# yangdongchao/RSTnet

Hardware: NVIDIA H100
Metric: codec_frames_per_s (higher is better)
Workload: dtype f32

## Files before the change

rstnet_b200/csrc/gemm_tc.cu:

```cuda
#include <cstdlib>

#include "common.cuh"
#include "tc_common.cuh"
#include "../../include/rstnet_b200.h"

namespace rstnet {
extern void count_launch();
using namespace tc;

constexpr int TC_BM = 128;
constexpr int TC_BKE = 32;
constexpr int TC_A_BYTES = TC_BM * 128;
constexpr int TC_CONSUMER_WARPS = 8;
constexpr int TC_THREADS = 32 * TC_CONSUMER_WARPS + 32;
constexpr int TC_CHUNK_STAGES = 4;

struct TcParams {
  float* C;
  float* C2;
  int act2;
  long long c_i_stride, c_o_stride, c_split_stride;
  const float* R;
  long long r_i_stride, r_o_stride, r_split_stride;
  const float* bias;
  const float* scale;
  int n_split;
  int I_out, O_out, N, Kc;
  int taps, tap_di, tap_do, o_mul, kchunks;
  int pre_act, post_act, i_tiles;
  int m_tiles, n_tiles;
};

template <int BN, int PREC>
struct TcCfg {
  static constexpr bool SPLIT = PREC == 0;
  static constexpr int B_BYTES = BN * 128;
  static constexpr int STAGE_BYTES = TC_A_BYTES + B_BYTES * (SPLIT ? 2 : 1);
  static constexpr int STAGES = (200 * 1024 / STAGE_BYTES) > 8 ? 8 : (200 * 1024 / STAGE_BYTES);
  static constexpr int SMEM_BYTES = STAGES * STAGE_BYTES + 1024  + 256 ;
};

__device__ __forceinline__ float tf32_rna(float x) {
  const uint32_t u = __float_as_uint(x);
  return __uint_as_float((x != x ? u | 0x00400000u : u + 0x1000u) & 0xFFFFE000u);
}
__device__ __forceinline__ float tf32_rna_lo(float x, float hi) {
  const float d = x - hi;
  return d != d ? 0.f : __uint_as_float((__float_as_uint(d) + 0x1000u) & 0xFFFFE000u);
}

__device__ __forceinline__ float act_tc(float x, int act) {
  if (act == ACT_ELU) return elu_fast(x);
  if (act == ACT_GELU) return gelu_f(x);
  return x;
}

template <bool SPLIT, bool PRE_ELU>
__device__ __forceinline__ void tc_build_a(uint32_t st, uint32_t a_row, uint32_t a_sw, uint32_t (&ah)[4][4], uint32_t (&al)[4][4]) {
#pragma unroll
  for (int k = 0; k < 4; ++k) {
#pragma unroll
    for (int e = 0; e < 4; ++e) {
      const uint32_t chunk = (uint32_t)(2 * k + (e >> 1));
      float v;
      asm volatile("ld.shared.f32 %0, [%1];" : "=f"(v) : "r"(st + a_row + (e & 1) * 1024u + ((chunk ^ a_sw) << 4)));
      if (PRE_ELU) {
        const float e = __expf(v) - 1.f;
        v = v > 0.f ? v : e;
      }
      if (SPLIT) {
        const bool nonfinite = !(fabsf(v) < INFINITY);
        const float h = nonfinite ? 0.f : __uint_as_float((__float_as_uint(v) + 0x1000u) & 0xFFFFE000u);
        const float d = v - h;
        ah[k][e] = __float_as_uint(h);
        al[k][e] = (__float_as_uint(d) + (nonfinite ? 0u : 0x1000u)) & 0xFFFFE000u;
      } else {
        ah[k][e] = __float_as_uint(tf32_rna(v));
      }
    }
  }
}

template <int BN, bool SPLIT>
__device__ __forceinline__ void tc_mma_stage(float (&d0)[BN / 2], float (&d1)[BN / 2], const uint32_t (&ah)[4][4],
                                             const uint32_t (&al)[4][4], uint64_t db, uint64_t dbl, bool first) {
#pragma unroll
  for (int k = 0; k < 4; ++k) {
    const uint32_t acc_in = (first && k == 0) ? 0u : 1u;
    wgmma_tf32_rs<BN>(d0, ah[k], db + (uint64_t)(2 * k), acc_in);
    if (SPLIT) {
      wgmma_tf32_rs<BN>(d1, al[k], db + (uint64_t)(2 * k), acc_in);
      wgmma_tf32_rs<BN>(d1, ah[k], dbl + (uint64_t)(2 * k), 1u);
    }
  }
}

template <int BN, int PREC, bool PRE_ELU>
__global__ void __launch_bounds__(TC_THREADS, 1)
gemm_tc_kernel(const __grid_constant__ CUtensorMap tmA, const __grid_constant__ CUtensorMap tmW,
               const __grid_constant__ CUtensorMap tmWlo, const TcParams p) {
  using Cfg = TcCfg<BN, PREC>;
  constexpr int S = Cfg::STAGES;
  constexpr int CH = TC_CHUNK_STAGES;
  constexpr int NR = BN / 2;
  extern __shared__ uint8_t smem_raw[];
  uint8_t* smem = smem_raw + ((1024u - (smem_u32(smem_raw) & 1023u)) & 1023u);
  uint64_t* full = reinterpret_cast<uint64_t*>(smem + S * Cfg::STAGE_BYTES);
  uint64_t* empty = full + S;
  const int warp = threadIdx.x / 32, lane = threadIdx.x % 32;
  const int total_k = p.taps * p.kchunks;
  const int total_tiles = p.m_tiles * p.n_tiles;

  if (threadIdx.x == 0) {
    for (int s = 0; s < S; ++s) {
      mbar_init(&full[s], 1);
      mbar_init(&empty[s], TC_CONSUMER_WARPS);
    }
    fence_barrier_init();
  }
  __syncthreads();

  if (warp == TC_CONSUMER_WARPS) {
    if (elect_one()) {
      tma_prefetch_desc(&tmA);
      tma_prefetch_desc(&tmW);
      if (Cfg::SPLIT) tma_prefetch_desc(&tmWlo);
      int g = 0;
      for (int t = blockIdx.x; t < total_tiles; t += gridDim.x) {
        const int nt = t % p.n_tiles, mt = t / p.n_tiles;
        const int i0 = (mt % p.i_tiles) * TC_BM, ot = mt / p.i_tiles, n0 = nt * BN;
        for (int kit = 0; kit < total_k; ++kit, ++g) {
          const int s = g % S;
          mbar_wait(&empty[s], ((g / S) & 1) ^ 1);
          const int tap = kit / p.kchunks, kc = kit % p.kchunks;
          uint8_t* st = smem + s * Cfg::STAGE_BYTES;
          mbar_arrive_expect_tx(&full[s], Cfg::STAGE_BYTES);
          tma_load_3d(st, &tmA, &full[s], kc * TC_BKE, i0 + tap * p.tap_di, ot * p.o_mul + tap * p.tap_do);
          tma_load_2d(st + TC_A_BYTES, &tmW, &full[s], kit * TC_BKE, n0);
          if (Cfg::SPLIT) tma_load_2d(st + TC_A_BYTES + Cfg::B_BYTES, &tmWlo, &full[s], kit * TC_BKE, n0);
        }
      }
    }
    return;
  }

  const int wg = warp / 4, wq = warp % 4, gq = lane / 4, tq = lane % 4;
  const int r0 = wg * 64 + wq * 16 + gq;
  const uint32_t a_row = (uint32_t)r0 * 128u + (uint32_t)tq * 4u, a_sw = (uint32_t)(r0 & 7);
  const uint32_t smem0 = smem_u32(smem);
  float acc[NR], d0[NR], d1[NR];
#pragma unroll
  for (int j = 0; j < NR; ++j) d0[j] = d1[j] = 0.f;
  int g = 0;
  for (int t = blockIdx.x; t < total_tiles; t += gridDim.x) {
    const int nt = t % p.n_tiles, mt = t / p.n_tiles;
    const int i0 = (mt % p.i_tiles) * TC_BM, ot = mt / p.i_tiles, n0 = nt * BN;
#pragma unroll
    for (int j = 0; j < NR; ++j) acc[j] = 0.f;
    for (int k0 = 0; k0 < total_k; k0 += CH) {
      const int nst = total_k - k0 < CH ? total_k - k0 : CH;
      for (int u = 0; u < nst; ++u, ++g) {
        const int s = g % S;
        mbar_wait(&full[s], (g / S) & 1);
        const uint32_t st = smem0 + (uint32_t)(s * Cfg::STAGE_BYTES);
        uint32_t ah[4][4], al[4][4];
        tc_build_a<Cfg::SPLIT, PRE_ELU>(st, a_row, a_sw, ah, al);
        const uint64_t db = gmma_desc_sw128(st + TC_A_BYTES);
        const uint64_t dbl = gmma_desc_sw128(st + TC_A_BYTES + Cfg::B_BYTES);
        wgmma_fence();
        tc_mma_stage<BN, Cfg::SPLIT>(d0, d1, ah, al, db, dbl, u == 0);
        wgmma_commit();
        wgmma_wait<0>();
        __syncwarp();
        if (lane == 0) mbar_arrive(&empty[s]);
      }
      fence_acc(d0);
      if (Cfg::SPLIT) fence_acc(d1);
#pragma unroll
      for (int j = 0; j < NR; ++j) acc[j] += Cfg::SPLIT ? d0[j] + d1[j] : d0[j];
    }
#pragma unroll
    for (int h = 0; h < 2; ++h) {
      const int i = i0 + r0 + 8 * h;
      if (i >= p.I_out) continue;
      float* crow = p.C + (long long)ot * p.c_o_stride + (long long)i * p.c_i_stride;
      float* crow2 = p.C2 ? p.C2 + (long long)ot * p.c_o_stride + (long long)i * p.c_i_stride : nullptr;
      const float* rrow = p.R ? p.R + (long long)ot * p.r_o_stride + (long long)i * p.r_i_stride : nullptr;
#pragma unroll
      for (int b = 0; b < BN / 8; ++b) {
        const int n = n0 + 8 * b + 2 * tq;
        if (n < p.N) {
          float2 v = make_float2(acc[4 * b + 2 * h], acc[4 * b + 2 * h + 1]);
          if (p.bias) {
            const float2 bb = *reinterpret_cast<const float2*>(p.bias + n);
            v.x += bb.x; v.y += bb.y;
          }
          if (p.scale) {
            const float2 ss = *reinterpret_cast<const float2*>(p.scale + n);
            v.x *= ss.x; v.y *= ss.y;
          }
          long long coff = n, roff = n;
          if (p.n_split > 0) {
            const int j = n / p.n_split, co = n % p.n_split;
            coff = (long long)j * p.c_split_stride + co;
            roff = (long long)j * p.r_split_stride + co;
          }
          if (rrow) {
            const float2 rr = *reinterpret_cast<const float2*>(rrow + roff);
            v.x += rr.x; v.y += rr.y;
          }
          if (crow2)
            *reinterpret_cast<float2*>(crow2 + coff) = make_float2(act_tc(v.x, p.act2), act_tc(v.y, p.act2));
          *reinterpret_cast<float2*>(crow + coff) = make_float2(act_tc(v.x, p.post_act), act_tc(v.y, p.post_act));
        }
      }
    }
  }
}

constexpr int RB_B_BYTES = 64 * 128;
constexpr int RB_STAGE_BYTES = TC_A_BYTES + 2 * RB_B_BYTES;
constexpr int RB_STAGES = 6;

struct RbParams {
  float* out;
  long long o_i_stride, o_o_stride;
  const float* b1;
  const float* b2;
  int I_out, i_tiles, m_tiles;
};

template <int C>
struct RbCfg {
  static constexpr int N1 = C / 2;
  static constexpr int KCH = C / 32;
  static constexpr int P1 = 3 * KCH;
  static constexpr int NS = C / 64;
  static constexpr int K2 = N1 / 32;
  static constexpr int H_BYTES = K2 * TC_A_BYTES;
  static constexpr int SMEM_BYTES = RB_STAGES * RB_STAGE_BYTES + H_BYTES + 1024  + 256 ;
  static constexpr bool ring_ok() {
    for (int j = 0; j < NS; ++j)
      for (int kc = 0; kc < KCH; ++kc)
        if ((P1 + j) % RB_STAGES == (2 * KCH + kc) % RB_STAGES) return false;
    return RB_STAGES >= KCH + NS;
  }
  static_assert(ring_ok(), "ring too small for the held residual stages");
  static_assert(K2 * 2 * RB_B_BYTES <= RB_STAGE_BYTES, "a phase-2 slice must fit one stage");
};

template <int C>
__global__ void __launch_bounds__(TC_THREADS, 1)
resblock_tc_kernel(const __grid_constant__ CUtensorMap tmY, const __grid_constant__ CUtensorMap tmW1,
                   const __grid_constant__ CUtensorMap tmW1lo, const __grid_constant__ CUtensorMap tmW2,
                   const __grid_constant__ CUtensorMap tmW2lo, const RbParams p) {
  using Cfg = RbCfg<C>;
  constexpr int S = RB_STAGES;
  constexpr int CH = TC_CHUNK_STAGES;
  constexpr int N1 = Cfg::N1, NR1 = N1 / 2, KCH = Cfg::KCH, P1 = Cfg::P1;
  extern __shared__ uint8_t smem_raw[];
  uint8_t* smem = smem_raw + ((1024u - (smem_u32(smem_raw) & 1023u)) & 1023u);
  uint8_t* hs = smem + S * RB_STAGE_BYTES;
  uint64_t* full = reinterpret_cast<uint64_t*>(hs + Cfg::H_BYTES);
  uint64_t* empty = full + S;
  const int warp = threadIdx.x / 32, lane = threadIdx.x % 32;

  if (threadIdx.x == 0) {
    for (int s = 0; s < S; ++s) {
      mbar_init(&full[s], 1);
      mbar_init(&empty[s], TC_CONSUMER_WARPS);
    }
    fence_barrier_init();
  }
  __syncthreads();

  if (warp == TC_CONSUMER_WARPS) {
    if (elect_one()) {
      tma_prefetch_desc(&tmY);
      tma_prefetch_desc(&tmW1);
      tma_prefetch_desc(&tmW1lo);
      tma_prefetch_desc(&tmW2);
      tma_prefetch_desc(&tmW2lo);
      int g = 0;
      for (int t = blockIdx.x; t < p.m_tiles; t += gridDim.x) {
        const int i0 = (t % p.i_tiles) * TC_BM, ot = t / p.i_tiles;
        for (int kit = 0; kit < P1; ++kit, ++g) {
          const int s = g % S;
          mbar_wait(&empty[s], ((g / S) & 1) ^ 1);
          const int tap = kit / KCH, kc = kit % KCH;
          uint8_t* st = smem + s * RB_STAGE_BYTES;
          mbar_arrive_expect_tx(&full[s], TC_A_BYTES + 2 * N1 * 128);
          tma_load_3d(st, &tmY, &full[s], kc * TC_BKE, i0, ot + tap);
          tma_load_2d(st + TC_A_BYTES, &tmW1, &full[s], kit * TC_BKE, 0);
          tma_load_2d(st + TC_A_BYTES + RB_B_BYTES, &tmW1lo, &full[s], kit * TC_BKE, 0);
        }
        for (int ns = 0; ns < Cfg::NS; ++ns, ++g) {
          const int s = g % S;
          mbar_wait(&empty[s], ((g / S) & 1) ^ 1);
          uint8_t* st = smem + s * RB_STAGE_BYTES;
          mbar_arrive_expect_tx(&full[s], Cfg::K2 * 2 * RB_B_BYTES);
#pragma unroll
          for (int kc = 0; kc < Cfg::K2; ++kc) {
            tma_load_2d(st + kc * 2 * RB_B_BYTES, &tmW2, &full[s], kc * TC_BKE, ns * 64);
            tma_load_2d(st + kc * 2 * RB_B_BYTES + RB_B_BYTES, &tmW2lo, &full[s], kc * TC_BKE, ns * 64);
          }
        }
      }
    }
    return;
  }

  const int wg = warp / 4, wq = warp % 4, gq = lane / 4, tq = lane % 4;
  const int r0 = wg * 64 + wq * 16 + gq;
  const uint32_t a_row = (uint32_t)r0 * 128u + (uint32_t)tq * 4u, a_sw = (uint32_t)(r0 & 7);
  const uint32_t smem0 = smem_u32(smem), hs0 = smem_u32(hs);
  int g = 0;
  for (int t = blockIdx.x; t < p.m_tiles; t += gridDim.x) {
    const int i0 = (t % p.i_tiles) * TC_BM, ot = t / p.i_tiles;
    const int g_res = g + 2 * KCH;
    {
      float acc[NR1], d0[NR1], d1[NR1];
#pragma unroll
      for (int j = 0; j < NR1; ++j) acc[j] = d0[j] = d1[j] = 0.f;
      for (int k0 = 0; k0 < P1; k0 += CH) {
        const int nst = P1 - k0 < CH ? P1 - k0 : CH;
        for (int u = 0; u < nst; ++u, ++g) {
          const int s = g % S;
          mbar_wait(&full[s], (g / S) & 1);
          const uint32_t st = smem0 + (uint32_t)(s * RB_STAGE_BYTES);
          uint32_t ah[4][4], al[4][4];
          tc_build_a<true, true>(st, a_row, a_sw, ah, al);
          wgmma_fence();
          tc_mma_stage<N1, true>(d0, d1, ah, al, gmma_desc_sw128(st + TC_A_BYTES), gmma_desc_sw128(st + TC_A_BYTES + RB_B_BYTES),
                                 u == 0);
          wgmma_commit();
          wgmma_wait<0>();
          __syncwarp();
          if (lane == 0 && k0 + u < 2 * KCH) mbar_arrive(&empty[s]);
        }
        fence_acc(d0);
        fence_acc(d1);
#pragma unroll
        for (int j = 0; j < NR1; ++j) acc[j] += d0[j] + d1[j];
      }
      named_bar_sync(1 + wg, 128);
#pragma unroll
      for (int hh = 0; hh < 2; ++hh) {
        const int r = r0 + 8 * hh;
#pragma unroll
        for (int b = 0; b < N1 / 8; ++b) {
          const int n = 8 * b + 2 * tq;
          const float2 bb = *reinterpret_cast<const float2*>(p.b1 + n);
          float2 v = make_float2(acc[4 * b + 2 * hh], acc[4 * b + 2 * hh + 1]);
          v.x += bb.x; v.y += bb.y;
          const uint32_t cc = (uint32_t)(n % 32);
          const uint32_t addr = hs0 + (uint32_t)(n / 32) * TC_A_BYTES + (uint32_t)r * 128u + (((cc >> 2) ^ (uint32_t)(r & 7)) << 4) +
                                (cc & 3u) * 4u;
          asm volatile("st.shared.v2.f32 [%0], {%1, %2};" ::"r"(addr), "f"(act_tc(v.x, ACT_ELU)), "f"(act_tc(v.y, ACT_ELU))
                       : "memory");
        }
      }
      named_bar_sync(1 + wg, 128);
    }
    for (int ns = 0; ns < Cfg::NS; ++ns, ++g) {
      const int s = g % S;
      mbar_wait(&full[s], (g / S) & 1);
      const uint32_t st = smem0 + (uint32_t)(s * RB_STAGE_BYTES);
      float acc[32], d0[32], d1[32];
#pragma unroll
      for (int j = 0; j < 32; ++j) d0[j] = d1[j] = 0.f;
#pragma unroll
      for (int kc = 0; kc < Cfg::K2; ++kc) {
        uint32_t ah[4][4], al[4][4];
        tc_build_a<true, false>(hs0 + (uint32_t)(kc * TC_A_BYTES), a_row, a_sw, ah, al);
        const uint32_t wst = st + (uint32_t)(kc * 2 * RB_B_BYTES);
        wgmma_fence();
        tc_mma_stage<64, true>(d0, d1, ah, al, gmma_desc_sw128(wst), gmma_desc_sw128(wst + RB_B_BYTES), kc == 0);
        wgmma_commit();
        wgmma_wait<0>();
      }
      __syncwarp();
      if (lane == 0) mbar_arrive(&empty[s]);
      fence_acc(d0);
      fence_acc(d1);
#pragma unroll
      for (int j = 0; j < 32; ++j) {
        acc[j] = 0.f;
        acc[j] += d0[j] + d1[j];
      }
#pragma unroll
      for (int hh = 0; hh < 2; ++hh) {
        const int r = r0 + 8 * hh;
        const int i = i0 + r;
        if (i >= p.I_out) continue;
        float* orow = p.out + (long long)ot * p.o_o_stride + (long long)i * p.o_i_stride;
#pragma unroll
        for (int b = 0; b < 8; ++b) {
          const int n = ns * 64 + 8 * b + 2 * tq;
          const float2 bb = *reinterpret_cast<const float2*>(p.b2 + n);
          float2 v = make_float2(acc[4 * b + 2 * hh], acc[4 * b + 2 * hh + 1]);
          v.x += bb.x; v.y += bb.y;
          const uint32_t cc = (uint32_t)(n % 32);
          const int rs = (g_res + n / 32) % S;
          const float2 rr = *reinterpret_cast<const float2*>(smem + rs * RB_STAGE_BYTES + r * 128 +
                                                             (((cc >> 2) ^ (uint32_t)(r & 7)) << 4) + (cc & 3u) * 4u);
          v.x += rr.x; v.y += rr.y;
          *reinterpret_cast<float2*>(orow + n) = make_float2(act_tc(v.x, ACT_ELU), act_tc(v.y, ACT_ELU));
        }
      }
      __syncwarp();
      if (lane == 0) {
        mbar_arrive(&empty[(g_res + 2 * ns) % S]);
        mbar_arrive(&empty[(g_res + 2 * ns + 1) % S]);
      }
    }
  }
}

typedef CUresult (*EncodeTiledFn)(CUtensorMap*, CUtensorMapDataType, cuuint32_t, void*, const cuuint64_t*, const cuuint64_t*,
                                  const cuuint32_t*, const cuuint32_t*, CUtensorMapInterleave, CUtensorMapSwizzle,
                                  CUtensorMapL2promotion, CUtensorMapFloatOOBfill);

static EncodeTiledFn get_encode_fn() {
  static EncodeTiledFn fn = nullptr;
  if (!fn) {
    void* p = nullptr;
    cudaDriverEntryPointQueryResult q;
    if (cudaGetDriverEntryPoint("cuTensorMapEncodeTiled", &p, cudaEnableDefault, &q) == cudaSuccess && p) fn = (EncodeTiledFn)p;
  }
  return fn;
}

}
using namespace rstnet;

struct rstnet_tc_plan {
  CUtensorMap tmA, tmW, tmWlo;
  TcParams p;
  dim3 grid;
  int bn, prec;
};

template <int BN, int PREC, bool PRE_ELU>
static int tc_launch(const rstnet_tc_plan* pl, cudaStream_t st) {
  using Cfg = TcCfg<BN, PREC>;
  static unsigned long long attr = 0;
  smem_optin(gemm_tc_kernel<BN, PREC, PRE_ELU>, Cfg::SMEM_BYTES, attr);
  gemm_tc_kernel<BN, PREC, PRE_ELU><<<pl->grid, TC_THREADS, Cfg::SMEM_BYTES, st>>>(pl->tmA, pl->tmW, pl->tmWlo, pl->p);
  count_launch();
  return check_launch("gemm_tc");
}

extern "C" int rstnet_tc_gemm_create(const rstnet_tc_gemm_desc* d, rstnet_tc_plan** out) {
  RSTNET_REQUIRE(d && out, "tc_gemm_create: null argument");
  RSTNET_REQUIRE(d->A && d->W && d->C, "tc_gemm_create: null tensor pointer");
  RSTNET_REQUIRE(d->precision != 0 || d->W_lo, "tc_gemm_create: precision 0 (3xTF32) needs W_lo");
  RSTNET_REQUIRE(d->Kc > 0 && d->Kc % TC_BKE == 0, "tc_gemm_create: Kc (%d) must be a multiple of %d", d->Kc, TC_BKE);
  RSTNET_REQUIRE(d->N > 0 && d->N % 4 == 0, "tc_gemm_create: N (%d) must be a multiple of 4", d->N);
  RSTNET_REQUIRE(d->taps >= 1 && d->I_out > 0 && d->O_out > 0, "tc_gemm_create: bad shape");
  RSTNET_REQUIRE(d->precision == 0 || d->precision == 1, "tc_gemm_create: precision must be 0 (3xTF32) or 1 (TF32)");
  RSTNET_REQUIRE(d->pre_act == ACT_NONE || d->pre_act == ACT_ELU, "tc_gemm_create: pre_act must be NONE or ELU (got %d)", d->pre_act);
  RSTNET_REQUIRE((uintptr_t)d->A % 16 == 0 && (uintptr_t)d->W % 16 == 0 && (uintptr_t)d->C % 16 == 0 &&
                     d->a_i_stride % 4 == 0 && d->a_o_stride % 4 == 0 && d->c_i_stride % 4 == 0 && d->c_o_stride % 4 == 0 &&
                     d->c_split_stride % 4 == 0 && d->n_split % 4 == 0,
                 "tc_gemm_create: 16-byte alignment required");
  EncodeTiledFn enc = get_encode_fn();
  RSTNET_REQUIRE(enc != nullptr, "tc_gemm_create: cuTensorMapEncodeTiled unavailable (no CUDA driver?)");
  rstnet_tc_plan* pl = new rstnet_tc_plan();
  const int N = d->N;
  const int sms = sm_count();
  pl->bn = N >= 64 ? 64 : 32;
  const int i_tiles = ceil_div(d->I_out, TC_BM);
  {
    const long long mt = (long long)i_tiles * d->O_out;
    const long long t64 = mt * ceil_div(N, 64), t32 = mt * ceil_div(N, 32);
    if (pl->bn == 64 && ((t32 + sms - 1) / sms) * 2 <= ((t64 + sms - 1) / sms) * 3) pl->bn = 32;
  }
  pl->prec = d->precision;
  {
    cuuint64_t gdim[3] = {(cuuint64_t)d->a_c_extent, (cuuint64_t)d->a_i_extent, (cuuint64_t)d->a_o_extent};
    cuuint64_t gstr[2] = {(cuuint64_t)d->a_i_stride * 4, (cuuint64_t)d->a_o_stride * 4};
    cuuint32_t box[3] = {TC_BKE, TC_BM, 1};
    cuuint32_t estr[3] = {1, 1, 1};
    CUresult r = enc(&pl->tmA, CU_TENSOR_MAP_DATA_TYPE_FLOAT32, 3, (void*)d->A, gdim, gstr, box, estr, CU_TENSOR_MAP_INTERLEAVE_NONE,
                     CU_TENSOR_MAP_SWIZZLE_128B, CU_TENSOR_MAP_L2_PROMOTION_L2_128B, CU_TENSOR_MAP_FLOAT_OOB_FILL_NONE);
    if (r != CUDA_SUCCESS) {
      delete pl;
      set_error("tc_gemm_create: cuTensorMapEncodeTiled(A) failed with %d", (int)r);
      return 3;
    }
  }
  {
    cuuint64_t gdim[2] = {(cuuint64_t)d->taps * d->Kc, (cuuint64_t)N};
    cuuint64_t gstr[1] = {(cuuint64_t)d->taps * d->Kc * 4};
    cuuint32_t box[2] = {TC_BKE, (cuuint32_t)pl->bn};
    cuuint32_t estr[2] = {1, 1};
    CUresult r = enc(&pl->tmW, CU_TENSOR_MAP_DATA_TYPE_FLOAT32, 2, (void*)d->W, gdim, gstr, box, estr, CU_TENSOR_MAP_INTERLEAVE_NONE,
                     CU_TENSOR_MAP_SWIZZLE_128B, CU_TENSOR_MAP_L2_PROMOTION_L2_256B, CU_TENSOR_MAP_FLOAT_OOB_FILL_NONE);
    if (r == CUDA_SUCCESS && d->W_lo)
      r = enc(&pl->tmWlo, CU_TENSOR_MAP_DATA_TYPE_FLOAT32, 2, (void*)d->W_lo, gdim, gstr, box, estr, CU_TENSOR_MAP_INTERLEAVE_NONE,
              CU_TENSOR_MAP_SWIZZLE_128B, CU_TENSOR_MAP_L2_PROMOTION_L2_256B, CU_TENSOR_MAP_FLOAT_OOB_FILL_NONE);
    else
      pl->tmWlo = pl->tmW;
    if (r != CUDA_SUCCESS) {
      delete pl;
      set_error("tc_gemm_create: cuTensorMapEncodeTiled(W) failed with %d", (int)r);
      return 3;
    }
  }
  TcParams& p = pl->p;
  p.C2 = d->C2; p.act2 = d->act2;
  p.C = d->C; p.c_i_stride = d->c_i_stride; p.c_o_stride = d->c_o_stride; p.c_split_stride = d->c_split_stride;
  p.R = d->R; p.r_i_stride = d->r_i_stride; p.r_o_stride = d->r_o_stride; p.r_split_stride = d->r_split_stride;
  p.bias = d->bias; p.scale = d->scale; p.n_split = d->n_split;
  p.I_out = d->I_out; p.O_out = d->O_out; p.N = N; p.Kc = d->Kc;
  p.taps = d->taps; p.tap_di = d->tap_di; p.tap_do = d->tap_do; p.o_mul = d->o_mul; p.kchunks = d->Kc / TC_BKE;
  p.pre_act = d->pre_act; p.post_act = d->post_act; p.i_tiles = i_tiles;
  p.m_tiles = i_tiles * d->O_out;
  p.n_tiles = ceil_div(N, pl->bn);
  const long long tiles = (long long)p.m_tiles * p.n_tiles;
  pl->grid = dim3((unsigned)(tiles < sms ? tiles : sms));
  *out = pl;
  return 0;
}

extern "C" int rstnet_tc_gemm_run(const rstnet_tc_plan* pl, rstnet_stream_t stream) {
  RSTNET_REQUIRE(pl != nullptr, "tc_gemm_run: null plan");
  cudaStream_t st = (cudaStream_t)stream;
  const bool elu = pl->p.pre_act == ACT_ELU;
  if (pl->prec == 0) {
    if (pl->bn == 64) return elu ? tc_launch<64, 0, true>(pl, st) : tc_launch<64, 0, false>(pl, st);
    return elu ? tc_launch<32, 0, true>(pl, st) : tc_launch<32, 0, false>(pl, st);
  }
  if (pl->bn == 64) return elu ? tc_launch<64, 1, true>(pl, st) : tc_launch<64, 1, false>(pl, st);
  return elu ? tc_launch<32, 1, true>(pl, st) : tc_launch<32, 1, false>(pl, st);
}

extern "C" void rstnet_tc_gemm_destroy(rstnet_tc_plan* pl) { delete pl; }

struct rstnet_tc_resblock_plan {
  CUtensorMap tmY, tmW1, tmW1lo, tmW2, tmW2lo;
  RbParams p;
  dim3 grid;
  int channels;
};

static int encode_2d(CUtensorMap* m, const float* base, int cols, int rows, int box_rows) {
  cuuint64_t gdim[2] = {(cuuint64_t)cols, (cuuint64_t)rows};
  cuuint64_t gstr[1] = {(cuuint64_t)cols * 4};
  cuuint32_t box[2] = {TC_BKE, (cuuint32_t)box_rows};
  cuuint32_t estr[2] = {1, 1};
  return (int)get_encode_fn()(m, CU_TENSOR_MAP_DATA_TYPE_FLOAT32, 2, (void*)base, gdim, gstr, box, estr, CU_TENSOR_MAP_INTERLEAVE_NONE,
                              CU_TENSOR_MAP_SWIZZLE_128B, CU_TENSOR_MAP_L2_PROMOTION_L2_256B, CU_TENSOR_MAP_FLOAT_OOB_FILL_NONE);
}

extern "C" int rstnet_tc_resblock_create(const rstnet_tc_resblock_desc* d, rstnet_tc_resblock_plan** out) {
  RSTNET_REQUIRE(d && out, "tc_resblock_create: null argument");
  RSTNET_REQUIRE(d->Y && d->W1 && d->W1_lo && d->b1 && d->W2 && d->W2_lo && d->b2 && d->out, "tc_resblock_create: null pointer");
  const int Cc = d->channels;
  RSTNET_REQUIRE(Cc == 64 || Cc == 128, "tc_resblock_create: channels must be 64 or 128 (got %d)", Cc);
  RSTNET_REQUIRE(d->I_out > 0 && d->O_out > 0 && d->y_rows >= d->O_out + 2, "tc_resblock_create: bad shape");
  RSTNET_REQUIRE((uintptr_t)d->Y % 16 == 0 && (uintptr_t)d->W1 % 16 == 0 && (uintptr_t)d->W1_lo % 16 == 0 && (uintptr_t)d->W2 % 16 == 0 &&
                     (uintptr_t)d->W2_lo % 16 == 0 && (uintptr_t)d->out % 16 == 0 && (uintptr_t)d->b1 % 8 == 0 &&
                     (uintptr_t)d->b2 % 8 == 0 && d->y_i_stride % 4 == 0 && d->y_o_stride % 4 == 0 && d->out_i_stride % 4 == 0 &&
                     d->out_o_stride % 4 == 0,
                 "tc_resblock_create: 16-byte alignment required");
  RSTNET_REQUIRE(get_encode_fn() != nullptr, "tc_resblock_create: cuTensorMapEncodeTiled unavailable (no CUDA driver?)");
  rstnet_tc_resblock_plan* pl = new rstnet_tc_resblock_plan();
  pl->channels = Cc;
  int r;
  {
    cuuint64_t gdim[3] = {(cuuint64_t)Cc, (cuuint64_t)d->I_out, (cuuint64_t)d->y_rows};
    cuuint64_t gstr[2] = {(cuuint64_t)d->y_i_stride * 4, (cuuint64_t)d->y_o_stride * 4};
    cuuint32_t box[3] = {TC_BKE, TC_BM, 1};
    cuuint32_t estr[3] = {1, 1, 1};
    r = (int)get_encode_fn()(&pl->tmY, CU_TENSOR_MAP_DATA_TYPE_FLOAT32, 3, (void*)d->Y, gdim, gstr, box, estr, CU_TENSOR_MAP_INTERLEAVE_NONE,
                             CU_TENSOR_MAP_SWIZZLE_128B, CU_TENSOR_MAP_L2_PROMOTION_L2_128B, CU_TENSOR_MAP_FLOAT_OOB_FILL_NONE);
  }
  if (r == CUDA_SUCCESS) r = encode_2d(&pl->tmW1, d->W1, 3 * Cc, Cc / 2, Cc / 2);
  if (r == CUDA_SUCCESS) r = encode_2d(&pl->tmW1lo, d->W1_lo, 3 * Cc, Cc / 2, Cc / 2);
  if (r == CUDA_SUCCESS) r = encode_2d(&pl->tmW2, d->W2, Cc / 2, Cc, 64);
  if (r == CUDA_SUCCESS) r = encode_2d(&pl->tmW2lo, d->W2_lo, Cc / 2, Cc, 64);
  if (r != CUDA_SUCCESS) {
    delete pl;
    set_error("tc_resblock_create: cuTensorMapEncodeTiled failed with %d", r);
    return 3;
  }
  RbParams& p = pl->p;
  p.out = d->out; p.o_i_stride = d->out_i_stride; p.o_o_stride = d->out_o_stride;
  p.b1 = d->b1; p.b2 = d->b2;
  p.I_out = d->I_out;
  p.i_tiles = ceil_div(d->I_out, TC_BM);
  p.m_tiles = p.i_tiles * d->O_out;
  const int sms = sm_count();
  pl->grid = dim3((unsigned)(p.m_tiles < sms ? p.m_tiles : sms));
  *out = pl;
  return 0;
}

template <int Cc>
static int rb_launch(const rstnet_tc_resblock_plan* pl, cudaStream_t st) {
  constexpr int smem = RbCfg<Cc>::SMEM_BYTES;
  static unsigned long long attr = 0;
  smem_optin(resblock_tc_kernel<Cc>, smem, attr);
  resblock_tc_kernel<Cc><<<pl->grid, TC_THREADS, smem, st>>>(pl->tmY, pl->tmW1, pl->tmW1lo, pl->tmW2, pl->tmW2lo, pl->p);
  count_launch();
  return check_launch("tc_resblock");
}

extern "C" int rstnet_tc_resblock_run(const rstnet_tc_resblock_plan* pl, rstnet_stream_t stream) {
  RSTNET_REQUIRE(pl != nullptr, "tc_resblock_run: null plan");
  cudaStream_t st = (cudaStream_t)stream;
  return pl->channels == 64 ? rb_launch<64>(pl, st) : rb_launch<128>(pl, st);
}

extern "C" void rstnet_tc_resblock_destroy(rstnet_tc_resblock_plan* pl) { delete pl; }
extern "C" int rstnet_tc_gemm_grid(const rstnet_tc_plan* pl, int32_t* gx, int32_t* gy, int32_t* bn) {
  if (!pl) return 1;
  *gx = pl->p.m_tiles; *gy = pl->p.n_tiles; *bn = pl->bn;
  return 0;
}

namespace rstnet {
__global__ void tf32_split_kernel(const float* __restrict__ x, float* __restrict__ hi, float* __restrict__ lo, long long n) {
  for (long long i = (long long)blockIdx.x * blockDim.x + threadIdx.x; i < n; i += (long long)gridDim.x * blockDim.x) {
    const float v = x[i], h = tf32_rna(v);
    hi[i] = h;
    lo[i] = tf32_rna_lo(v, h);
  }
}
}

extern "C" int rstnet_tf32_split_f32(const float* x, float* hi, float* lo, int64_t n, rstnet_stream_t stream) {
  RSTNET_REQUIRE(x && hi && lo, "tf32_split: null pointer");
  if (n <= 0) return 0;
  int g = ceil_div(n, 256);
  if (g > sm_count() * 8) g = sm_count() * 8;
  rstnet::tf32_split_kernel<<<g, 256, 0, (cudaStream_t)stream>>>(x, hi, lo, n);
  count_launch();
  return check_launch("tf32_split");
}
```

Baseline: 42930.

## Add split-K with workspace and finalize kernel for small-tile TC GEMMs

```diff
diff --git a/rstnet_b200/csrc/gemm_tc.cu b/rstnet_b200/csrc/gemm_tc.cu
--- a/rstnet_b200/csrc/gemm_tc.cu
+++ b/rstnet_b200/csrc/gemm_tc.cu
@@ -1,4 +1,6 @@
 #include <cstdlib>
+#include <map>
+#include <mutex>
 
 #include "common.cuh"
 #include "tc_common.cuh"
@@ -29,6 +31,8 @@
   int taps, tap_di, tap_do, o_mul, kchunks;
   int pre_act, post_act, i_tiles;
   int m_tiles, n_tiles;
+  float* ws;
+  int ksplit, kspan;
 };
 
 template <int BN, int PREC>
@@ -53,6 +57,30 @@
   if (act == ACT_ELU) return elu_fast(x);
   if (act == ACT_GELU) return gelu_f(x);
   return x;
+}
+
+__device__ __forceinline__ void tc_store_pair(const TcParams& p, float* crow, float* crow2, const float* rrow, int n, float2 v) {
+  if (p.bias) {
+    const float2 bb = *reinterpret_cast<const float2*>(p.bias + n);
+    v.x += bb.x; v.y += bb.y;
+  }
+  if (p.scale) {
+    const float2 ss = *reinterpret_cast<const float2*>(p.scale + n);
+    v.x *= ss.x; v.y *= ss.y;
+  }
+  long long coff = n, roff = n;
+  if (p.n_split > 0) {
+    const int j = n / p.n_split, co = n % p.n_split;
+    coff = (long long)j * p.c_split_stride + co;
+    roff = (long long)j * p.r_split_stride + co;
+  }
+  if (rrow) {
+    const float2 rr = *reinterpret_cast<const float2*>(rrow + roff);
+    v.x += rr.x; v.y += rr.y;
+  }
+  if (crow2)
+    *reinterpret_cast<float2*>(crow2 + coff) = make_float2(act_tc(v.x, p.act2), act_tc(v.y, p.act2));
+  *reinterpret_cast<float2*>(crow + coff) = make_float2(act_tc(v.x, p.post_act), act_tc(v.y, p.post_act));
 }
 
 template <bool SPLIT, bool PRE_ELU>
@@ -109,7 +137,8 @@
   uint64_t* empty = full + S;
   const int warp = threadIdx.x / 32, lane = threadIdx.x % 32;
   const int total_k = p.taps * p.kchunks;
-  const int total_tiles = p.m_tiles * p.n_tiles;
+  const int mn_tiles = p.m_tiles * p.n_tiles;
+  const int total_tiles = mn_tiles * p.ksplit;
 
   if (threadIdx.x == 0) {
     for (int s = 0; s < S; ++s) {
@@ -127,9 +156,11 @@
       if (Cfg::SPLIT) tma_prefetch_desc(&tmWlo);
       int g = 0;
       for (int t = blockIdx.x; t < total_tiles; t += gridDim.x) {
-        const int nt = t % p.n_tiles, mt = t / p.n_tiles;
+        const int tmn = t % mn_tiles, kb = t / mn_tiles * p.kspan;
+        const int ke = total_k - kb < p.kspan ? total_k : kb + p.kspan;
+        const int nt = tmn % p.n_tiles, mt = tmn / p.n_tiles;
         const int i0 = (mt % p.i_tiles) * TC_BM, ot = mt / p.i_tiles, n0 = nt * BN;
-        for (int kit = 0; kit < total_k; ++kit, ++g) {
+        for (int kit = kb; kit < ke; ++kit, ++g) {
           const int s = g % S;
           mbar_wait(&empty[s], ((g / S) & 1) ^ 1);
           const int tap = kit / p.kchunks, kc = kit % p.kchunks;
@@ -153,12 +184,14 @@
   for (int j = 0; j < NR; ++j) d0[j] = d1[j] = 0.f;
   int g = 0;
   for (int t = blockIdx.x; t < total_tiles; t += gridDim.x) {
-    const int nt = t % p.n_tiles, mt = t / p.n_tiles;
+    const int tmn = t % mn_tiles, kb = t / mn_tiles * p.kspan;
+    const int ke = total_k - kb < p.kspan ? total_k : kb + p.kspan;
+    const int nt = tmn % p.n_tiles, mt = tmn / p.n_tiles;
     const int i0 = (mt % p.i_tiles) * TC_BM, ot = mt / p.i_tiles, n0 = nt * BN;
 #pragma unroll
     for (int j = 0; j < NR; ++j) acc[j] = 0.f;
-    for (int k0 = 0; k0 < total_k; k0 += CH) {
-      const int nst = total_k - k0 < CH ? total_k - k0 : CH;
+    for (int k0 = kb; k0 < ke; k0 += CH) {
+      const int nst = ke - k0 < CH ? ke - k0 : CH;
       for (int u = 0; u < nst; ++u, ++g) {
         const int s = g % S;
         mbar_wait(&full[s], (g / S) & 1);
@@ -176,9 +209,26 @@
       }
       fence_acc(d0);
       if (Cfg::SPLIT) fence_acc(d1);
-#pragma unroll
-      for (int j = 0; j < NR; ++j) acc[j] += Cfg::SPLIT ? d0[j] + d1[j] : d0[j];
-    }
+      if (p.ws) {
+#pragma unroll
+        for (int h = 0; h < 2; ++h) {
+          const int i = i0 + r0 + 8 * h;
+          if (i >= p.I_out) continue;
+          float* wrow = p.ws + (((long long)(k0 / CH) * p.O_out + ot) * p.I_out + i) * p.N;
+#pragma unroll
+          for (int b = 0; b < BN / 8; ++b) {
+            const int n = n0 + 8 * b + 2 * tq, j = 4 * b + 2 * h;
+            if (n < p.N)
+              *reinterpret_cast<float2*>(wrow + n) =
+                  Cfg::SPLIT ? make_float2(d0[j] + d1[j], d0[j + 1] + d1[j + 1]) : make_float2(d0[j], d0[j + 1]);
+          }
+        }
+      } else {
+#pragma unroll
+        for (int j = 0; j < NR; ++j) acc[j] += Cfg::SPLIT ? d0[j] + d1[j] : d0[j];
+      }
+    }
+    if (p.ws) continue;
 #pragma unroll
     for (int h = 0; h < 2; ++h) {
       const int i = i0 + r0 + 8 * h;
@@ -189,32 +239,30 @@
 #pragma unroll
       for (int b = 0; b < BN / 8; ++b) {
         const int n = n0 + 8 * b + 2 * tq;
-        if (n < p.N) {
-          float2 v = make_float2(acc[4 * b + 2 * h], acc[4 * b + 2 * h + 1]);
-          if (p.bias) {
-            const float2 bb = *reinterpret_cast<const float2*>(p.bias + n);
-            v.x += bb.x; v.y += bb.y;
-          }
-          if (p.scale) {
-            const float2 ss = *reinterpret_cast<const float2*>(p.scale + n);
-            v.x *= ss.x; v.y *= ss.y;
-          }
-          long long coff = n, roff = n;
-          if (p.n_split > 0) {
-            const int j = n / p.n_split, co = n % p.n_split;
-            coff = (long long)j * p.c_split_stride + co;
-            roff = (long long)j * p.r_split_stride + co;
-          }
-          if (rrow) {
-            const float2 rr = *reinterpret_cast<const float2*>(rrow + roff);
-            v.x += rr.x; v.y += rr.y;
-          }
-          if (crow2)
-            *reinterpret_cast<float2*>(crow2 + coff) = make_float2(act_tc(v.x, p.act2), act_tc(v.y, p.act2));
-          *reinterpret_cast<float2*>(crow + coff) = make_float2(act_tc(v.x, p.post_act), act_tc(v.y, p.post_act));
-        }
-      }
-    }
+        if (n < p.N)
+          tc_store_pair(p, crow, crow2, rrow, n, make_float2(acc[4 * b + 2 * h], acc[4 * b + 2 * h + 1]));
+      }
+    }
+  }
+}
+
+__global__ void tc_finalize_kernel(const TcParams p, int nchunks) {
+  const long long pairs = (long long)p.O_out * p.I_out * (p.N / 2);
+  const long long plane = (long long)p.O_out * p.I_out * p.N;
+  for (long long q = (long long)blockIdx.x * blockDim.x + threadIdx.x; q < pairs; q += (long long)gridDim.x * blockDim.x) {
+    const int n = (int)(q % (p.N / 2)) * 2;
+    const long long row = q / (p.N / 2);
+    const int i = (int)(row % p.I_out), ot = (int)(row / p.I_out);
+    const float* w = p.ws + row * p.N + n;
+    float2 acc = make_float2(0.f, 0.f);
+    for (int c = 0; c < nchunks; ++c) {
+      const float2 v = *reinterpret_cast<const float2*>(w + c * plane);
+      acc.x += v.x; acc.y += v.y;
+    }
+    float* crow = p.C + (long long)ot * p.c_o_stride + (long long)i * p.c_i_stride;
+    float* crow2 = p.C2 ? p.C2 + (long long)ot * p.c_o_stride + (long long)i * p.c_i_stride : nullptr;
+    const float* rrow = p.R ? p.R + (long long)ot * p.r_o_stride + (long long)i * p.r_i_stride : nullptr;
+    tc_store_pair(p, crow, crow2, rrow, n, acc);
   }
 }
 
@@ -434,11 +482,42 @@
 }
 using namespace rstnet;
 
+static std::mutex g_ws_mu;
+static std::multimap<size_t, float*> g_ws_free;
+
+static float* ws_take(size_t bytes, size_t* got) {
+  {
+    std::lock_guard<std::mutex> lk(g_ws_mu);
+    auto it = g_ws_free.lower_bound(bytes);
+    if (it != g_ws_free.end()) {
+      float* p = it->second;
+      *got = it->first;
+      g_ws_free.erase(it);
+      return p;
+    }
+  }
+  float* p = nullptr;
+  if (cudaMalloc(&p, bytes) != cudaSuccess) {
+    cudaGetLastError();
+    return nullptr;
+  }
+  *got = bytes;
+  return p;
+}
+
+static void ws_give(float* p, size_t bytes) {
+  std::lock_guard<std::mutex> lk(g_ws_mu);
+  g_ws_free.emplace(bytes, p);
+}
+
 struct rstnet_tc_plan {
   CUtensorMap tmA, tmW, tmWlo;
   TcParams p;
   dim3 grid;
   int bn, prec;
+  int nchunks;
+  size_t ws_bytes;
+  dim3 fin_grid;
 };
 
 template <int BN, int PREC, bool PRE_ELU>
@@ -448,7 +527,11 @@
   smem_optin(gemm_tc_kernel<BN, PREC, PRE_ELU>, Cfg::SMEM_BYTES, attr);
   gemm_tc_kernel<BN, PREC, PRE_ELU><<<pl->grid, TC_THREADS, Cfg::SMEM_BYTES, st>>>(pl->tmA, pl->tmW, pl->tmWlo, pl->p);
   count_launch();
-  return check_launch("gemm_tc");
+  if (int r = check_launch("gemm_tc")) return r;
+  if (!pl->p.ws) return 0;
+  tc_finalize_kernel<<<pl->fin_grid, 256, 0, st>>>(pl->p, pl->nchunks);
+  count_launch();
+  return check_launch("gemm_tc_finalize");
 }
 
 extern "C" int rstnet_tc_gemm_create(const rstnet_tc_gemm_desc* d, rstnet_tc_plan** out) {
@@ -519,7 +602,29 @@
   p.m_tiles = i_tiles * d->O_out;
   p.n_tiles = ceil_div(N, pl->bn);
   const long long tiles = (long long)p.m_tiles * p.n_tiles;
-  pl->grid = dim3((unsigned)(tiles < sms ? tiles : sms));
+  const int total_k = p.taps * p.kchunks;
+  pl->nchunks = ceil_div(total_k, TC_CHUNK_STAGES);
+  p.ws = nullptr;
+  p.ksplit = 1;
+  p.kspan = total_k;
+  if (tiles * 2 <= sms && pl->nchunks >= 2) {
+    const int want = (int)(sms / tiles) < pl->nchunks ? (int)(sms / tiles) : pl->nchunks;
+    const int per = ceil_div(pl->nchunks, want);
+    p.ksplit = ceil_div(pl->nchunks, per);
+    p.kspan = per * TC_CHUNK_STAGES;
+    const size_t bytes = (size_t)pl->nchunks * d->O_out * d->I_out * N * sizeof(float);
+    p.ws = ws_take(bytes, &pl->ws_bytes);
+    if (!p.ws) {
+      delete pl;
+      set_error("tc_gemm_create: cudaMalloc of the %zu-byte K-split workspace failed", bytes);
+      return 2;
+    }
+    const long long pairs = (long long)d->O_out * d->I_out * (N / 2);
+    const long long fb = (pairs + 255) / 256;
+    pl->fin_grid = dim3((unsigned)(fb < 8LL * sms ? fb : 8LL * sms));
+  }
+  const long long ctas = tiles * p.ksplit;
+  pl->grid = dim3((unsigned)(ctas < sms ? ctas : sms));
   *out = pl;
   return 0;
 }
@@ -536,7 +641,10 @@
   return elu ? tc_launch<32, 1, true>(pl, st) : tc_launch<32, 1, false>(pl, st);
 }
 
-extern "C" void rstnet_tc_gemm_destroy(rstnet_tc_plan* pl) { delete pl; }
+extern "C" void rstnet_tc_gemm_destroy(rstnet_tc_plan* pl) {
+  if (pl && pl->p.ws) ws_give(pl->p.ws, pl->ws_bytes);
+  delete pl;
+}
 
 struct rstnet_tc_resblock_plan {
   CUtensorMap tmY, tmW1, tmW1lo, tmW2, tmW2lo;
```

Measured after the change: 43860, median of 6. +2.2%, better.
